# ascentai/diy-gym

Measured on AMD Instinct MI355X. Metric: env steps/sec (whole node), higher is better.
Workload: dtype f32; 1 GPU; ur_high_5 x 16384 envs per GPU; envs_total=16384, substeps=2, auto_reset=True, launch=hipGraph replay of 8-step segments, parallelism=independent env shards x1, no collective, envs_per_wavefront=64, lds_bytes_per_workgroup=160512, parity=vs the C oracle only; parity with pybullet itself is UNPINNED (DESIGN.md 4)

## Files before the change

### diy_gym_amd/backend.py

```python
import collections
import ctypes
import os

import numpy as np
import torch

_HERE = os.path.dirname(os.path.abspath(__file__))
LIB_PATH = os.path.join(_HERE, 'csrc', 'libdiygym_hip.so')

_lib = None

_c_i32p = ctypes.POINTER(ctypes.c_int32)
_c_f64p = ctypes.POINTER(ctypes.c_double)
_vp = ctypes.c_void_p


class JointSelector(ctypes.Structure):
    _fields_ = [('frame', ctypes.c_int32), ('flags', ctypes.c_int32), ('link_mask', ctypes.c_uint64), ('frame_mask', ctypes.c_uint64),
                ('rigid', ctypes.c_float * 10)]


class AccelSelector(ctypes.Structure):
    _fields_ = [('frame', ctypes.c_int32), ('com', ctypes.c_int32), ('pos', ctypes.c_float * 3), ('quat', ctypes.c_float * 4)]

# ... 32 lines not shown
    'dg_world_link_states': (ctypes.c_int32, [_vp, _vp, _c_i32p, _c_i32p, ctypes.c_int32, ctypes.c_int32, _vp, _vp]),
    'dg_world_reset_base_state': (ctypes.c_int32, [_vp, _vp, ctypes.c_int32, _vp, _vp, _vp, _vp, _vp, _vp]),
    'dg_world_joint_wrench': (ctypes.c_int32, [_vp, _vp, ctypes.c_int32, ctypes.POINTER(JointSelector), ctypes.c_int32, _vp, _vp]),
    'dg_world_joint_efforts': (ctypes.c_int32, [_vp, _vp, ctypes.c_int32, _vp, _vp]),
    'dg_world_link_accelerations': (ctypes.c_int32, [_vp, _vp, ctypes.c_int32, ctypes.POINTER(AccelSelector), ctypes.c_int32, _vp, _vp]),
    'dg_world_task_space': (ctypes.c_int32, [_vp, _vp, ctypes.c_int32, ctypes.c_int32, ctypes.POINTER(ctypes.c_float), ctypes.c_int32, _vp, _vp, _vp, _vp,
                                             ctypes.c_float, _vp, _vp, _vp, _vp, _vp, _vp, _vp, _vp]),
    'dg_world_forward_dynamics': (ctypes.c_int32, [_vp, _vp, ctypes.c_int32, _vp, _vp, _vp, ctypes.c_int32, _vp, _vp, _vp]),
    'dg_world_rollout': (ctypes.c_int32, [_vp, _vp, ctypes.c_int32, ctypes.c_int32, ctypes.POINTER(ctypes.c_float), ctypes.c_int32, ctypes.c_int32, ctypes.c_float,
                                          ctypes.c_int32, _vp, _vp, _vp, _vp, _vp, _vp, _vp, _vp]),
    'dg_world_dynamics_derivatives': (ctypes.c_int32, [_vp, _vp, ctypes.c_int32, ctypes.c_int32, _vp, _vp, _vp, ctypes.c_int32, _vp, _vp, _vp, _vp, _vp, _vp, _vp, _vp]),
    'dg_world_rollout_feedback': (ctypes.c_int32, [_vp, _vp, ctypes.c_int32, ctypes.c_int32, ctypes.POINTER(ctypes.c_float), ctypes.c_int32, ctypes.c_int32, ctypes.c_float,
                                                   ctypes.c_int32, _vp, _vp, _vp, _vp, _vp, _vp, _vp, _vp, _vp, _vp, _vp, _vp, _vp, _vp, _vp]),
    'dg_world_inertial_parameters': (ctypes.c_int32, [_vp, _vp, ctypes.c_int32, ctypes.c_int32, _vp, _vp]),
    'dg_world_id_regressor': (ctypes.c_int32, [_vp, _vp, ctypes.c_int32, ctypes.c_int32, _vp, _vp, _vp, _vp, _vp, _vp, _vp, _vp, _vp, _vp]),
    'dg_world_lq_backward': (ctypes.c_int32, [_vp, ctypes.c_int32, ctypes.c_int32, ctypes.c_int32, ctypes.c_int32, ctypes.c_int32, ctypes.c_double,
                                              _vp, _vp, _vp, _vp, _vp, _vp, _vp, _vp, _vp, _vp, _vp, _vp, _vp, _vp, _vp]),
    'dg_world_closest_scratch_floats': (ctypes.c_int64, [_vp]),
    'dg_world_closest': (ctypes.c_int32, [_vp, _vp, ctypes.c_int32, ctypes.c_int32, ctypes.c_int32, ctypes.c_int32, ctypes.c_float, ctypes.c_int32, _vp,
                                          _vp, _vp, _vp, _vp, _vp, _vp]),
    'dg_world_set_render_diag': (ctypes.c_int32, [_vp, ctypes.c_int32]),
    'dg_world_set_diag_buffer': (ctypes.c_int32, [_vp, _vp]),
    'dg_world_set_skip_counter': (ctypes.c_int32, [_vp, _vp]),
    'dg_world_set_profile_buffer': (ctypes.c_int32, [_vp, _vp]),
    'dg_debug_plan': (ctypes.c_int32, [_c_i32p, ctypes.c_int64, _c_f64p, ctypes.c_int64, ctypes.c_int32, ctypes.c_int32, _c_i32p, _c_i32p,
                                       ctypes.c_int64]),
}


def load_library(path=None):
    global _lib
    if _lib is not None and path is None:
        return _lib
    path = path or LIB_PATH
    if not os.path.isfile(path):
        raise RuntimeError('HIP library not built: %s is missing. Run `python -c "import __graft_entry__ as g; g.build()"` '
                           '(or `make -j8 -C diy_gym_amd/csrc`).  There is no CPU fallback.' % path)
    lib = ctypes.CDLL(path)
    for name, (res, args) in SYMBOLS.items():
        fn = getattr(lib, name)
        fn.restype = res
        fn.argtypes = args
    _lib = lib
    return lib


# ... 159 lines not shown
class HipBackend:
    def __init__(self, layout, num_envs, device=None, seed=0, env_index_base=0):
        if not torch.cuda.is_available():
            raise RuntimeError('diy_gym_amd needs a ROCm GPU (torch.cuda.is_available() is False); there is no CPU fallback')
        self.lib = load_library()
        self.layout = layout
        self.num_envs = int(num_envs)
        self.device = torch.device(device if device is not None else 'cuda:0')
        if self.device.type != 'cuda':
            raise RuntimeError('diy_gym_amd runs on ROCm devices only, got %s' % self.device)
        dev_index = self.device.index if self.device.index is not None else torch.cuda.current_device()
        self.device = torch.device('cuda', dev_index)
        self.stride = ((self.num_envs + 63) // 64) * 64
        I, F = layout.I, layout.F
        handle = _vp()
        rc = self.lib.dg_world_create(I.ctypes.data_as(_c_i32p), I.size, F.ctypes.data_as(_c_f64p), F.size, self.num_envs,
                                      self.stride, dev_index, ctypes.c_uint64(seed), ctypes.c_int64(env_index_base),
                                      ctypes.byref(handle))
        self._check(rc)
        self.handle = handle
        dims = (ctypes.c_int32 * 8)()
        self._check(self.lib.dg_world_dims(self.handle, dims))
        self.state_dim, self.act_dim, self.obs_dim, self.rew_dim, self.term_dim, self.n_links, self.lds_bytes, self.lanes = list(dims)
        B, dev = self.num_envs, self.device
        with torch.cuda.device(dev):
            self.state = torch.zeros((self.state_dim, self.stride), dtype=torch.float32, device=dev)
            self.act = torch.zeros((B, max(self.act_dim, 1)), dtype=torch.float32, device=dev)
            self.obs = torch.zeros((B, max(self.obs_dim, 1)), dtype=torch.float32, device=dev)
            self.rew = torch.zeros((B, max(self.rew_dim, 1)), dtype=torch.float32, device=dev)
            self.term = torch.zeros((B, max(self.term_dim, 1)), dtype=torch.uint8, device=dev)
            self.rew_sum = torch.zeros((B, ), dtype=torch.float32, device=dev)
            self.term_flag = torch.zeros((B, ), dtype=torch.uint8, device=dev)
        self._ray_scratch, self._ray_out = None, {}
        self._dyn_out = {}
        self._contact_out = {}
        self._contact_force_out, self._net_contact_out = {}, {}
        self._closest_scratch, self._closest_out = None, {}
        self._closest_k = {}
        self._ik_list_cache = {}
        self._link_states_out = {}
        self._joint_wrench_out = {}
        self._link_accel_out = {}
        self._link_accel_sel = {}
        self._check(self.lib.dg_world_init_state(self.handle, _ptr(self.state), self._stream()))

    def _stream(self):
# ... 918 lines not shown
```

### diy_gym_amd/csrc/dg_api.hip

```cpp
#include <hip/hip_runtime.h>

#include <cmath>
#include <cstdarg>
#include <cstdio>
#include <cstdlib>
#include <cstring>
#include <memory>
#include <string>
#include <vector>

#include "../../include/diygym_hip.h"
#include "dg_launch.h"
#include "dg_plan.h"
#define DG_DEFINE_RENDER_KERNEL
#include "dg_render.h"
#include "dg_raycast.h"
#include "dg_dynq.h"
#include "dg_ikq.h"
#include "dg_jointq.h"
#include "dg_accelq.h"
#include "dg_taskq.h"
#include "dg_fdq.h"
#include "dg_ddq.h"
#include "dg_regq.h"
// ... 192 lines not shown
  if (w->par) snprintf(buf, sizeof buf, "step_kernel_par (4 wavefronts per 64 envs)");
  else snprintf(buf, sizeof buf, "step_kernel<%d>", w->lanes);
  return buf;
}

int32_t dg_world_dims(const dg_world* w, int32_t dims[8]) {
  if (!w || !dims) return fail(DG_ERR_ARG, "null argument");
  dims[0] = w->sc.state_dim; dims[1] = w->sc.act_dim; dims[2] = w->sc.obs_dim; dims[3] = w->sc.rew_dim; dims[4] = w->sc.term_dim;
  dims[5] = w->sc.nl; dims[6] = w->lds_bytes; dims[7] = w->lanes;
  return DG_OK;
}
int32_t dg_world_get_motor_cfg(const dg_world* w, double* cfg) {
  if (!w || !cfg) return fail(DG_ERR_ARG, "null argument");
  for (int k = 0; k < 3 * w->sc.nl; k++) cfg[k] = w->mt.v[k];
  return DG_OK;
}
int32_t dg_world_set_motor_cfg(dg_world* w, const double* cfg) {
  if (!w || !cfg) return fail(DG_ERR_ARG, "null argument");
  for (int k = 0; k < 3 * w->sc.nl; k++) w->mt.v[k] = (float)cfg[k];
  return DG_OK;
}
int32_t dg_world_set_diag_buffer(dg_world* w, int32_t* diag) { if (!w) return fail(DG_ERR_ARG, "null world"); w->diag = diag; return DG_OK; }
int32_t dg_world_set_skip_counter(dg_world* w, int32_t* skipped) { if (!w) return fail(DG_ERR_ARG, "null world"); w->sc.skip_count = skipped; return DG_OK; }

int32_t dg_world_init_state(dg_world* w, float* state, void* stream) {
  if (!w || !state) return fail(DG_ERR_ARG, "null argument");
  DG_ON_DEVICE(w->device);
  hipLaunchKernelGGL(init_state_kernel, dim3((w->stride + 255) / 256), dim3(256), 0, (hipStream_t)stream, w->d_init, state, w->sc.state_dim, w->stride);
  HIP_TRY(hipGetLastError());
  return DG_OK;
}

int32_t dg_world_reset(dg_world* w, float* state, const uint8_t* mask, float* obs, void* stream) {
  if (!w || !state) return fail(DG_ERR_ARG, "null argument");
  if (!(w->par && w->sc.hot_start == 1 && !w->no_par_reset)) return launch(w, stream, &LaunchTable::reset, state, mask, obs);
  DG_ON_DEVICE(w->device);
  launch_table(w->lanes, w->mf).step_par(grid_of(w), w->lds_bytes, (hipStream_t)stream, false, w->sc, w->mt, state, nullptr, 0ull, obs, nullptr, nullptr, nullptr, nullptr, nullptr, nullptr, mask, 1);
  HIP_TRY(hipGetLastError());
  return DG_OK;
}

int32_t dg_world_step(dg_world* w, float* state, const float* actions, uint64_t update_mask, float* obs, float* rew, uint8_t* term,
                      float* rew_sum, uint8_t* term_flag, void* stream) {
  if (!w || !state) return fail(DG_ERR_ARG, "null argument");
  if (w->sc.act_dim > 0 && update_mask != 0 && !actions) return fail(DG_ERR_ARG, "update_mask selects controller addons but actions is NULL");
  DG_ON_DEVICE(w->device);
// ... 649 lines not shown
```

### diy_gym_amd/csrc/dg_kernels.h

```cpp
#pragma once
#include "dg_device.h"
#include "../../include/diygym_scene.h"
#include "../../include/diygym_hip.h"

namespace dg {

#define DG_MAX_LINKS 64
#define DG_MAX_BODIES 192

#define DG_CONSTANT __attribute__((address_space(4)))
typedef const int32_t DG_CONSTANT* cip;
typedef const float DG_CONSTANT* cfp;

struct DevScene {
  cip BI, LI, FI, SI, PI, GI, OI, IL;
  cfp BF, LF, FF, SF, PF, OF, FL, HF;
  cip PLB;
  int split_pgs;
  int early_dyn;
  int coll_split, cont2_off;
  int coll_wave;
  cfp GD;
  cip AM;
  cip SD;
  cip PD;
  cip PLL;
  int32_t nba;
  int32_t no_sliced_reset;
  int32_t no_minv_slices;
  int32_t nsha;
  int32_t debug_keep_ext;
  int32_t no_chain_rows;
  int32_t warm_off;
  float* hull_ws;
  int32_t ncons; cip KI; cfp KF;
  int32_t nb, nl, nfr, nsh, npairs, ngroups, nops, act_dim, obs_dim, rew_dim, term_dim, substeps, iters, hot_start, ik_iters;
  int32_t state_dim, addon_off, max_contacts, term_mode, n_term_groups;
  int32_t tr_off, tr_slots, cont_off, nv_max, total_slots, ab_stride;
  int32_t nt, dv_base, dense;
  int32_t crow_tail;
  int32_t helper_body;
  int32_t reg_body[2];
  int32_t num_envs, stride;
  uint64_t seed; int64_t env_base;
  float h, gx, gy, gz;
  float hm;
  int32_t np_skip;
  cfp RH;
  int32_t* skip_count;
};
struct MotorTable { float v[DG_MAX_LINKS * 3]; };

enum { PLB_R0 = 0, PLB_MINV, PLB_DV, PLB_NV, PLB_CHAIN , PLB_STRIDE };
enum { PLL_POSE = 0, PLL_MROW, PLL_IAACC , PLL_STRIDE };
enum { AW_E = 0, AW_R = 9, AW_V = 12, AW_PA = 18, AW_U = 24, AW_D = 30, AW_UU = 31, AW_STRIDE = 32 };
enum { AB_V = 0, AB_A = 6, AB_FIXED_STRIDE = 12, AB_IA = 12, AB_PA = 33, AB_L = 39, AB_FLOAT_STRIDE = 60 };
enum { CL_PAIR = 0, CL_P = 1, CL_N = 4, CL_DIST = 7, CL_KEY = 8, CL_DVA = 9, CL_NVA = 10, CL_DVB = 11, CL_NVB = 12, CL_MU = 13, CL_STRIDE = 14 };
enum { MR_B = 0, MR_ACC, MR_LO_B, MR_LO_ACC, MR_HI_B, MR_HI_ACC, MR_STRIDE };

constexpr int envs_per_wave(int lanes) { return lanes > 0 ? lanes : (lanes < 0 ? -lanes : 64); }

template <int LANES>
DGD float* workspace_of(const DevScene& sc, float* smem, float* gws, int lane) {
  if constexpr (LANES > 0) return smem + lane;
  else return gws + (size_t)blockIdx.x * (size_t)sc.total_slots * envs_per_wave(LANES) + lane;
}

template <int LANES>
struct Lane {
  const DevScene& sc;
// ... 313 lines not shown
        float rhs[6] = {-p0.a.x, -p0.a.y, -p0.a.z, -p0.l.x, -p0.l.y, -p0.l.z}, x[6];
        if (jdof < 0) {
#pragma unroll
          for (int k = 0; k < 6; k++) rhs[k] = (k == col) ? 1.0f : 0.0f;
        }
        chol6_solve(Lb, rhs, x);
        a0c.a = v3(x[0], x[1], x[2]); a0c.l = v3(x[3], x[4], x[5]);
#pragma unroll
        for (int k = 0; k < 6; k++) L(mo + col * nv + k) = x[k];
      }
      for (int i = 0; i <= jdof; i++) {
        int gl = first + i, par = li(gl)[DG_LI_PARENT]; int o = aw(i);
        S6 ap = par < 0 ? a0c : L6(aw(par - first) + AW_V);
        S6 a1 = xmotion(LM(o + AW_E), L3(o + AW_R), ap);
        float qdd = (L(o + AW_UU) - dot(L6(o + AW_U), a1)) / L(o + AW_D);
        L6set(o + AW_V, a1 + subspace(gl) * qdd);
        L(mo + col * nv + nb6 + i) = qdd;
      }
    }
    for (int r = 0; r < nv; r++) for (int c = r + 1; c < nv; c++) L(mo + r * nv + c) = L(mo + c * nv + r);
    prof.stamp(4 );
  }

  template <int N, class PROF_T>
  DGD void dynamics_chain(int b, PROF_T& prof) const {
    cip B = bi(b); const int first = B[DG_BI_FIRST_LINK], n = B[DG_BI_N_LINKS], mo = plb(b)[PLB_MINV]; const float h = sc.h;
    const M3 R0 = LR(plb(b)[PLB_R0]); const V3 gb = tmul(R0, v3(sc.gx, sc.gy, sc.gz));
    const float ka = ang_damping(b);
    const S6 zero6 = {v3(0.f, 0.f, 0.f), v3(0.f, 0.f, 0.f)};
    M3 E[N]; V3 r[N]; S6 v[N], pA[N], U[N], Sx[N]; float dinv[N], u[N], qd[N];
    S6 vp = zero6;
#pragma unroll
    for (int i = 0; i < N; i++) {
      E[i] = R0; r[i] = v3(0.f, 0.f, 0.f); v[i] = zero6; pA[i] = zero6; U[i] = zero6; Sx[i] = zero6; dinv[i] = 0.f; u[i] = 0.f; qd[i] = 0.f;
      if (i < n) {
        const int gl = first + i, lo = li(gl)[DG_LI_STATE_OFF]; cfp f = lf(gl);
        const float q = S(lo + DG_LS_Q); qd[i] = S(lo + DG_LS_QD);
        M3 Rpc; joint_xform(gl, q, Rpc, r[i]); E[i] = transpose(Rpc); Sx[i] = subspace(gl);
        v[i] = xmotion(E[i], r[i], vp) + Sx[i] * qd[i]; vp = v[i];
        float lm; V3 c; Sym3 Ic; link_inertia(gl, lm, c, Ic); (void)f;
        const AI I = rigid_inertia(lm, c, Ic);
        pA[i] = crf(v[i], mul(I, v[i])) - damping_force(lm, c, Ic, v[i], ka);
      }
    }
    AI carry; bool have = false;
#pragma unroll
    for (int i = N - 1; i >= 0; i--) {
      if (i < n) {
        const int gl = first + i, lo = li(gl)[DG_LI_STATE_OFF]; cfp f = lf(gl);
        const float tau = S(lo + DG_LS_TORQUE) - f[DG_LF_DAMPING] * qd[i];
        AI IA; { float lm; V3 lc; Sym3 lI; link_inertia(gl, lm, lc, lI); IA = rigid_inertia(lm, lc, lI); }
        if (have) {
          IA.I.xx += carry.I.xx; IA.I.xy += carry.I.xy; IA.I.xz += carry.I.xz; IA.I.yy += carry.I.yy; IA.I.yz += carry.I.yz; IA.I.zz += carry.I.zz;
          IA.M.xx += carry.M.xx; IA.M.xy += carry.M.xy; IA.M.xz += carry.M.xz; IA.M.yy += carry.M.yy; IA.M.yz += carry.M.yz; IA.M.zz += carry.M.zz;
#pragma unroll
          for (int k = 0; k < 9; k++) IA.H.m[k] += carry.H.m[k];
        }
        U[i] = mul(IA, Sx[i]); const float d = dot(Sx[i], U[i]); dinv[i] = 1.0f / d; u[i] = tau - dot(Sx[i], pA[i]);
        if (i > 0) {
          const float di = dinv[i]; const S6 Ui = U[i];
          AI Ia = IA;
          Ia.I.xx -= Ui.a.x * Ui.a.x * di; Ia.I.xy -= Ui.a.x * Ui.a.y * di; Ia.I.xz -= Ui.a.x * Ui.a.z * di;
          Ia.I.yy -= Ui.a.y * Ui.a.y * di; Ia.I.yz -= Ui.a.y * Ui.a.z * di; Ia.I.zz -= Ui.a.z * Ui.a.z * di;
          Ia.M.xx -= Ui.l.x * Ui.l.x * di; Ia.M.xy -= Ui.l.x * Ui.l.y * di; Ia.M.xz -= Ui.l.x * Ui.l.z * di;
          Ia.M.yy -= Ui.l.y * Ui.l.y * di; Ia.M.yz -= Ui.l.y * Ui.l.z * di; Ia.M.zz -= Ui.l.z * Ui.l.z * di;
          const float ua[3] = {Ui.a.x, Ui.a.y, Ui.a.z}, ul[3] = {Ui.l.x, Ui.l.y, Ui.l.z};
#pragma unroll
          for (int a = 0; a < 3; a++)
#pragma unroll
            for (int c2 = 0; c2 < 3; c2++) Ia.H.m[3 * a + c2] -= ua[a] * ul[c2] * di;
          const S6 c = crm(v[i], Sx[i] * qd[i]);
          const S6 pa = pA[i] + mul(Ia, c) + Ui * (u[i] * di);
          carry = to_parent(Ia, E[i], r[i]); have = true;
          pA[i - 1] = pA[i - 1] + xforce_to_parent(E[i], r[i], pa);
        }
      }
    }
    S6 ap; ap.a = v3(0.f, 0.f, 0.f); ap.l = -gb;
#pragma unroll
    for (int i = 0; i < N; i++) {
      if (i < n) {
        const S6 a1 = xmotion(E[i], r[i], ap) + crm(v[i], Sx[i] * qd[i]);
        const float qdd = (u[i] - dot(U[i], a1)) * dinv[i];
        ap = a1 + Sx[i] * qdd;
        Sset(li(first + i)[DG_LI_STATE_OFF] + DG_LS_QD, qd[i] + h * qdd);
      }
    }
    prof.stamp(3 );
#pragma unroll
    for (int col = 0; col < N; col++) {
      if (col < n) {
        S6 p[N]; float uu[N];
#pragma unroll
        for (int i = 0; i < N; i++) { p[i] = zero6; uu[i] = 0.f; }
#pragma unroll
        for (int i = col; i >= 0; i--) {
          uu[i] = (i == col ? 1.0f : 0.0f) - dot(Sx[i], p[i]);
          if (i > 0) p[i - 1] = p[i - 1] + xforce_to_parent(E[i], r[i], p[i] + U[i] * (uu[i] * dinv[i]));
        }
        S6 a = zero6;
#pragma unroll
        for (int i = 0; i < N; i++) {
          if (i < n) {
            const S6 a1 = xmotion(E[i], r[i], a);
            const float qdd = (uu[i] - dot(U[i], a1)) * dinv[i];
            a = a1 + Sx[i] * qdd;
            L(mo + col * n + i) = qdd;
          }
        }
      }
    }
// ... 139 lines not shown
```

### diy_gym_amd/csrc/dg_plan.h

```cpp
#pragma once
#include <string>
#include <vector>

#include "dg_kernels.h"

namespace dg {

#define DG_PLAN_SWITCHES(X) \
  X(DG_MAX_LANES, max_lanes, "32|16|8|4|1: envs per wavefront to start from; any value also switches the automatic narrowing off") \
  X(DG_NO_NARROW_MODES, no_narrow_modes, "never below 16 envs per wavefront") \
  X(DG_NO_WAVE_ENV, no_wave_env, "never one env per wavefront") \
  X(DG_NO_SLICED_GLOBAL, no_sliced_global, "global workspace with 64 envs per wavefront instead of 16") \
  X(DG_NO_HELPER_WAVE, no_helper_wave, "single-wavefront step kernel") \
  X(DG_NO_COLLIDE_WAVE, no_collide_wave, "the main wavefront runs the narrow phase itself") \
  X(DG_NO_COLLIDE_SPLIT, no_collide_split, "one narrow-phase wavefront instead of two") \
  X(DG_NO_EARLY_DYNAMICS, no_early_dynamics, "the first substep's dynamics wait for the update ops") \
  X(DG_NO_SPLIT_SWEEPS, no_split_sweeps, "the main wavefront sweeps both arms") \
  X(DG_NO_SPLIT_CONTACTS, no_split_contacts, "contact rows stay on the main wavefront when the sweeps are split") \
  X(DG_NO_REG_ROWS, no_reg_rows, "sliced sweeps keep their rows in LDS") \
  X(DG_NO_FULL_IK, no_full_ik, "the general register-resident IK instead of the packed six-axis solve") \
  X(DG_NO_MINV_SLICES, no_minv_slices, "M^-1 columns by one lane per env") \
  X(DG_NO_CHAIN_ROWS, no_chain_rows, "contact rows between two register-chain bodies pair by pair") \
  X(DG_NO_SLICED_RESET, no_sliced_reset, "masked resets through the one-lane-per-env reset kernel") \
  X(DG_NO_PAR_RESET, no_par_reset, "masked resets of four-wavefront scenes through the one-wavefront reset kernel") \
  X(DG_DEBUG_KEEP_EXT, debug_keep_ext, "external wrenches and joint torques are not cleared at the end of a step") \
  X(DG_RENDER_NO_CULL, render_no_cull, "render: every shape tested for every pixel group (render diag bit 0)") \
  X(DG_RENDER_DIAG, render_diag, "render: initial value of the dg_world_set_render_diag flags") \
  X(DG_RENDER_WPE, render_wpe, "render: 1|3 wavefronts per SIMD builds of the render kernel instead of 2")

struct Switch {
  bool set = false;
  int value = 0;
  explicit operator bool() const { return set; }
};
struct PlanSwitches {
#define X(name, field, doc) Switch field;
  DG_PLAN_SWITCHES(X)
#undef X
  Switch no_np_skip;
};
PlanSwitches plan_switches_from_env();

struct WorldPlan {
  int lanes = 64, lds_bytes = 0;
  bool par = false;
  bool mf = false;
  bool no_par_reset = false;
  int render_diag = 0, render_wpe = 2;
  size_t gws_floats = 0;
  size_t hull_ws_floats = 0;
  std::vector<int32_t> table;
  size_t pd_off = 0, gd_off = 0, sd_off = 0, am_off = 0, rh_off = 0;
  std::vector<int32_t> blob_i;
  std::vector<float> blob_f;
  MotorTable mt;
  std::vector<float> init;
  DevScene sc;
  std::string error;
};

int plan_world(const int32_t* I, int64_t n_i, const double* F, int64_t n_f, int num_envs, int env_stride, int cu_count, uint64_t seed,
               int64_t env_index_base, const PlanSwitches& sw, WorldPlan& out);
// ... 3 lines not shown
```

### diy_gym_amd/csrc/dg_plan.hip

```cpp
#include "dg_plan.h"

#include <algorithm>
#include <cmath>
#include <cstdarg>
#include <cstdio>
#include <cstdlib>
#include <cstring>

#include "dg_solver.h"

namespace dg {

PlanSwitches plan_switches_from_env() {
  PlanSwitches s;
#define X(name, field, doc) if (const char* v = getenv(#name)) { s.field.set = true; s.field.value = atoi(v); }
  DG_PLAN_SWITCHES(X)
#undef X
  if (const char* v = getenv("DG_NO_NP_SKIP")) { s.no_np_skip.set = true; s.no_np_skip.value = atoi(v); }
  return s;
}

namespace {

const int LDS_MAX = 160 * 1024;

const char* check_blob(const int32_t* I, int64_t n_i, int64_t n_f) {
  struct T { int off, count_idx, stride; bool is_f; const char* name; };
  const T tables[] = {
    {DG_H_OFF_BODY_I, DG_H_N_BODIES, DG_BI_STRIDE, false, "body ints"}, {DG_H_OFF_LINK_I, DG_H_N_LINKS, DG_LI_STRIDE, false, "link ints"},
    {DG_H_OFF_FRAME_I, DG_H_N_FRAMES, DG_FI_STRIDE, false, "frame ints"}, {DG_H_OFF_SHAPE_I, DG_H_N_SHAPES, DG_SI_STRIDE, false, "shape ints"},
    {DG_H_OFF_PAIR_I, DG_H_N_PAIRS, DG_PI_STRIDE, false, "pairs"}, {DG_H_OFF_GROUP_I, DG_H_N_GROUPS, DG_GI_STRIDE, false, "pair groups"},
    {DG_H_OFF_CAMERA_I, DG_H_N_CAMERAS, DG_CI_STRIDE, false, "camera ints"}, {DG_H_OFF_OP_I, DG_H_N_OPS, DG_OI_STRIDE, false, "op ints"},
    {DG_H_OFF_ILIST, DG_H_N_ILIST, 1, false, "int list"},
    {DG_H_OFF_BODY_F, DG_H_N_BODIES, DG_BF_STRIDE, true, "body floats"}, {DG_H_OFF_LINK_F, DG_H_N_LINKS, DG_LF_STRIDE, true, "link floats"},
    {DG_H_OFF_FRAME_F, DG_H_N_FRAMES, DG_FF_STRIDE, true, "frame floats"}, {DG_H_OFF_SHAPE_F, DG_H_N_SHAPES, DG_SF_STRIDE, true, "shape floats"},
    {DG_H_OFF_POINT_F, DG_H_N_POINTS, 3, true, "hull points"}, {DG_H_OFF_PLANE_F, DG_H_N_PLANES, 4, true, "hull planes"},
    {DG_H_OFF_CAMERA_F, DG_H_N_CAMERAS, DG_CF_STRIDE, true, "camera floats"}, {DG_H_OFF_OP_F, DG_H_N_OPS, DG_OF_STRIDE, true, "op floats"},
    {DG_H_OFF_FLIST, DG_H_N_FLIST, 1, true, "float list"},
    {DG_H_OFF_CONS_I, DG_H_N_CONSTRAINTS, DG_KI_STRIDE, false, "constraint ints"}, {DG_H_OFF_CONS_F, DG_H_N_CONSTRAINTS, DG_KF_STRIDE, true, "constraint floats"}};
  for (const T& t : tables) {
    const int64_t off = I[t.off], cnt = I[t.count_idx], lim = t.is_f ? n_f : n_i;
// ... 251 lines not shown
    }
  }
  sc.early_dyn = 0;
  if (sc.coll_wave && !sw.no_early_dynamics) {
    bool ok = true, long_update = false;
    for (int op = 0; op < nops; op++) {
      const int32_t* oi = OI + op * DG_OI_STRIDE; const int code = oi[DG_OI_CODE];
      if (code == DG_OP_IK_CONTROL) long_update = true;
      if (code == DG_OP_EXTERNAL_FORCE || code == DG_OP_PROPELLOR || code == DG_OP_ADMITTANCE || (code == DG_OP_JOINT_CONTROL && oi[DG_OI_FLAGS] == DG_JC_TORQUE)) ok = false;
    }
    sc.early_dyn = (ok && long_update) ? 1 : 0;
  }
  sc.np_skip = 0;
  if (sc.coll_wave && sc.coll_split && sc.split_pgs > 0 && ncons == 0 && sc.substeps >= 2 && !sw.no_np_skip && sc.total_slots * 64 * 4 <= LDS_MAX) {
    bool ok = sc.reg_body[0] >= 0 && sc.reg_body[1] == sc.helper_body;
    for (int k = 0; k < 2 && ok; k++) {
      const int32_t* B = BI + sc.reg_body[k] * DG_BI_STRIDE; const int first = B[DG_BI_FIRST_LINK];
      ok = is_fixed(B) && B[DG_BI_N_LINKS] == 6 && PLB[sc.reg_body[k] * PLB_STRIDE + PLB_CHAIN];
      for (int i = 0; i < 6 && ok; i++) ok = LI[(first + i) * DG_LI_STRIDE + DG_LI_TYPE] == 0;
    }
    for (int b = 0; b < nb && ok; b++) if (!is_static(BI + b * DG_BI_STRIDE) && b != sc.reg_body[0] && b != sc.reg_body[1]) ok = false;
    sc.np_skip = ok ? 1 : 0;
  }
  memset(&out.mt, 0, sizeof out.mt);
  for (int l = 0; l < nl; l++) { out.mt.v[3 * l] = 0.f; out.mt.v[3 * l + 1] = 1.f; out.mt.v[3 * l + 2] = -(float)F[DG_HF_DEFAULT_MOTOR_IMPULSE]; }
  for (int op = 0; op < nops; op++) {
    const int32_t* oi = OI + op * DG_OI_STRIDE;
    if (oi[DG_OI_CODE] == DG_OP_ADMITTANCE) for (int k = 0; k < oi[DG_OI_N]; k++) out.mt.v[3 * (I[I[DG_H_OFF_ILIST] + oi[DG_OI_ILIST] + k]) + 2] = 0.f;
  }
  std::vector<float>& init = out.init; init.assign((size_t)sc.state_dim, 0.f);
  const double* BF = F + I[DG_H_OFF_BODY_F];
  for (int b = 0; b < nb; b++) {
    const int so = BI[b * DG_BI_STRIDE + DG_BI_STATE_OFF]; if (so < 0) continue;
    for (int k = 0; k < 3; k++) init[so + DG_BS_POS + k] = (float)BF[b * DG_BF_STRIDE + DG_BF_INIT_POS + k];
    for (int k = 0; k < 4; k++) init[so + DG_BS_QUAT + k] = (float)BF[b * DG_BF_STRIDE + DG_BF_INIT_QUAT + k];
  }
  for (int op = 0; op < nops; op++) {
    const int32_t* oi = OI + op * DG_OI_STRIDE;
    if (oi[DG_OI_CODE] == DG_OP_RANDOMIZE_COLOR) {
      float* tx = init.data() + sc.addon_off + oi[DG_OI_STATE_OFF];
      for (int k = 0; k < 3; k++) tx[DG_TX_A + k] = tx[DG_TX_B + k] = (float)BF[oi[DG_OI_BODY] * DG_BF_STRIDE + DG_BF_COLOR + k];
      tx[DG_TX_FREQ] = 1.f; tx[DG_TX_KIND] = (float)DG_TEX_FLAT;
      continue;
    }
    if (oi[DG_OI_CODE] != DG_OP_RANDOMIZE_DYNAMICS) continue;
    const int so = sc.addon_off + oi[DG_OI_STATE_OFF];
// ... 8 lines not shown
```

### diy_gym_amd/csrc/dg_solver.h

```cpp
#pragma once
#include "dg_kernels.h"
#include "dg_hull.h"

namespace dg {

enum { PS_UPDATE = 0, PS_KIN, PS_COLLIDE, PS_ABA, PS_MINV, PS_ROWS, PS_PGS, PS_INTEGRATE, PS_OUTPUT, PS_PGS_MOTOR, PS_PGS_LIMIT, PS_PGS_CONTACT, PS_COUNT,
       PS_ROW = PS_COUNT + 12  };
template <bool PROF> struct Prof;
template <> struct Prof<false> { DGD void start() {} DGD void stamp(int) {} };
template <> struct Prof<true> {
  unsigned long long last, acc[PS_COUNT];
  DGD void start() { _Pragma("unroll") for (int k = 0; k < PS_COUNT; k++) acc[k] = 0ull; last = __builtin_amdgcn_s_memtime(); }
  DGD void stamp(int id) {
    unsigned long long t = __builtin_amdgcn_s_memtime();
    _Pragma("unroll") for (int k = 0; k < PS_COUNT; k++) if (k == id) acc[k] += t - last;
    last = t;
  }
};

struct WShape { int type, body, glink; M3 R; V3 p; float prm0, prm1, prm2, mu; int poff, npts; };

template <int LANES>
DGD void shape_world(const Lane<LANES>& ln, int sh, WShape& o) {
  cip si = ln.sc.SI + sh * DG_SI_STRIDE; cfp sf = ln.sc.SF + sh * DG_SF_STRIDE;
// ... 1822 lines not shown
template <int LANES>
DGD bool substep_contact_free(const Lane<LANES>& ln) {
  const DevScene& sc = ln.sc;
  if (sc.split_pgs <= 0 || sc.ncons > 0) return false;
  if (ln.bi(sc.reg_body[0])[DG_BI_N_LINKS] != 6 || ln.bi(sc.helper_body)[DG_BI_N_LINKS] != 6) return false;
  float cnt = ln.L(sc.cont_off);
  if (sc.coll_split) cnt = fmaxf(cnt, ln.L(sc.cont2_off));
  return !__any(cnt > 0.f);
}
template <int LANES>
DGD bool substep_np_skip(const Lane<LANES>& ln, bool prev_fused) {
  const DevScene& sc = ln.sc;
  if (!sc.np_skip || !prev_fused) return false;
  const int xo = split_slots(sc);
  const float clr = fminf(ln.L(xo + NPS_CLEAR), ln.L(xo + NPS_CLEAR + 1)), d = ln.L(xo + NPS_MOVE0) + ln.L(xo + NPS_MOVE1);
  return __all(clr > __builtin_fmaf(d, 1.0f + 0x1p-10f, 1e-4f));
}
template <int LANES>
DGD void np_skip_follow(const Lane<LANES>& ln, int which, int list) {
  const int xo = split_slots(ln.sc);
  ln.L(list) = 0.f;
  ln.L(xo + NPS_CLEAR + which) = ln.L(xo + NPS_CLEAR + which) - (ln.L(xo + NPS_MOVE0) + ln.L(xo + NPS_MOVE1));
}
template <int LANES, bool PROF>
DGD void fused_free_halves(const Lane<LANES>& ln, int wave, Prof<PROF>& prof) {
  constexpr int RN = 6;
  const DevScene& sc = ln.sc; const float h = sc.h, lerp = sc.HF[DG_HF_LIMIT_ERP], vmax = sc.HF[DG_HF_MAX_COORD_VEL];
  const float thr_abs = sqrtf(sc.HF[DG_HF_RESIDUAL_THRESHOLD]);
  int lane = threadIdx.x & 63; asm volatile("" : "+v"(lane));
  const int half = lane >> 5, el = (lane & 31) + 32 * wave;
  float* const col = ln.lds - (threadIdx.x & 63) + el;
  const int envl = (int)blockIdx.x * 64 + el; const bool exists = envl < sc.num_envs;
  const bool store = (__ballot(ln.valid) >> el) & 1ull;
  float* const st = ln.st - ln.env + (exists ? envl : sc.num_envs - 1);
  const size_t stride = sc.stride;
  const int b0 = sc.reg_body[0], b1 = sc.helper_body;
  const int f0 = ln.bi(b0)[DG_BI_FIRST_LINK], f1 = ln.bi(b1)[DG_BI_FIRST_LINK];
  const int mvo = half ? ln.plb(b1)[PLB_MINV] : ln.plb(b0)[PLB_MINV];
  const float* const cm = col + (size_t)mvo * 64;
  int lo[RN]; float q[RN], qd[RN], tp[RN], tv[RN];
#pragma unroll
  for (int i = 0; i < RN; i++) {
    const int lo0 = ln.li(f0 + i)[DG_LI_STATE_OFF], lo1 = ln.li(f1 + i)[DG_LI_STATE_OFF]; lo[i] = half ? lo1 : lo0;
    q[i] = st[(lo[i] + DG_LS_Q) * stride]; qd[i] = st[(lo[i] + DG_LS_QD) * stride];
    tp[i] = st[(lo[i] + DG_LS_TARGET_POS) * stride]; tv[i] = st[(lo[i] + DG_LS_TARGET_VEL) * stride];
  }
// ... 89 lines not shown
  uint64_t limit_rows = 0ull;
  const float thr = sc.HF[DG_HF_RESIDUAL_THRESHOLD]; const int rs = crow_stride(sc.crow_tail);
  const bool early = PAR && sc.early_dyn && index == 0;
  constexpr int EPW = envs_per_wave(LANES), SLN = SLICED ? 64 / EPW : 1, SLOG = SLN == 64 ? 6 : SLN == 16 ? 4 : SLN == 8 ? 3 : SLN == 4 ? 2 : SLN == 2 ? 1 : 0;
  const int qlane = threadIdx.x & 63, qsl = qlane & (SLN - 1), qe = qlane >> SLOG;
  const int qenv = blockIdx.x * EPW + qe; const bool qvalid = qenv < sc.num_envs; const int qec = qvalid ? qenv : sc.num_envs - 1;
  const Lane<LANES> lq(sc, ln.mt, SLICED ? ln.lds - qlane + qe : ln.lds, SLICED ? ln.st - ln.env + qec : ln.st, SLICED ? qec : ln.env, SLICED ? qvalid : ln.valid);
  if (primary) {
  if (index == sc.substeps - 1 && !early) for (int b = 0; b < sc.nba; b++) if (b != hb) save_prev_velocities(ln, b);
  if (!early && !(PAR && np_skip)) for (int b = 0; b < sc.nba; b++) if (b != hb) ln.kinematics(b);
  }
  if (PAR) __syncthreads();
  prof.stamp(PS_KIN);
  if constexpr (SLICED) collide<LANES, 64, SLN>(lq, 0, 0x7fffffff, -1, qsl);
  const bool own_collide = !(PAR && sc.coll_wave);
  if (primary) {
  if constexpr (SLICED) ncont = (int)ln.L(sc.cont_off);
  else if (own_collide) ncont = collide<LANES, FULLWAVE ? 64 : (PAR ? 64 : 0)>(ln);
  prof.stamp(PS_COLLIDE);
  }
  if (!early) for (int b = 0; b < sc.nba; b++) {
    if (b == hb || (ln.fixed(b) && ln.bi(b)[DG_BI_N_LINKS] == 0)) continue;
    const int mslices = (SLICED && !ln.plb(b)[PLB_CHAIN] && !sc.no_minv_slices) ? ln.minv_slices(b, SLN) : 0;
    if (primary) { if (ln.plb(b)[PLB_CHAIN]) ln.template dynamics_chain<6>(b, prof); else ln.dynamics(b, prof, mslices > 0); }
    if constexpr (SLICED) { if (mslices > 0) { lq.minv_sliced(b, qsl, mslices, SLN); prof.stamp(4 ); } }
    if (primary) {
      const int dvo = ln.plb(b)[PLB_DV], nv = ln.plb(b)[PLB_NV];
      for (int k = 0; k < nv; k++) ln.L(dvo + k) = 0.f;
    }
  }
  if (primary) {
  if (PAR) __syncthreads();
  if constexpr (PAR) { fused = substep_contact_free(ln); if (fused) fused_free_halves(ln, 0, prof); }
  if (!fused) {
  if (!own_collide) {
    ncont = (int)ln.L(sc.cont_off);
    if (sc.coll_split) {
      const int nb2 = (int)ln.L(sc.cont2_off);
      if (__any(nb2 > 0)) {
        for (int j = 0; j < sc.max_contacts; j++) {
          if (!__any(j < nb2)) break;
          if (j < nb2 && ncont + j < sc.max_contacts) {
            float* dst = ln.lds + (sc.cont_off + 1 + (ncont + j) * CL_STRIDE) * envs_per_wave(LANES);
#pragma unroll
            for (int k = 0; k < CL_KEY + 1; k++) dst[k * envs_per_wave(LANES)] = ln.L(sc.cont2_off + 1 + j * CL_STRIDE + k);
          }
        }
// ... 238 lines not shown
    int32_t* d = diag_out + (size_t)DG_DIAG_STRIDE * ln.env;
    d[DG_DIAG_CONTACTS] = ncont; d[DG_DIAG_PGS_ITERS] = iters_done;
    if (index == 0) { d[DG_DIAG_PGS_ITERS_FIRST] = iters_done; d[DG_DIAG_CONTACTS_FIRST] = ncont; }
  };
  if (primary) {
  store_warm_cache(ln, ncont, wave_max_cont);
  if (diag_out && ln.valid && !fused) write_diag();
  for (int b = 0; b < sc.nba; b++) if (!((split_now || fused) && b == hb) && !(fused && b == sc.reg_body[0])) integrate_body(ln, b);
  }
  if (PAR) __syncthreads();
  if constexpr (PAR) {
    if (fused && diag_out && ln.valid) { iters_done = (int)ln.L(split_slots(sc)); write_diag(); }
  }
  return fused;
}

template <int LANES>
DGD bool helper_substep(const Lane<LANES>& ln, bool early, bool last, bool np_skip) {
  const DevScene& sc = ln.sc; const int hb = sc.helper_body; Prof<false> none;
  if (last && !early) save_prev_velocities(ln, hb);
  if (!early && !np_skip) ln.kinematics(hb);
  __syncthreads();
  if (!early) {
    ln.template dynamics_chain<6>(hb, none);
    const int dvo = ln.plb(hb)[PLB_DV], nv = ln.plb(hb)[PLB_NV]; for (int k = 0; k < nv; k++) ln.L(dvo + k) = 0.f;
  }
  __syncthreads();
  if (substep_contact_free(ln)) { fused_free_halves(ln, 1, none); __syncthreads();  return true; }
  uint64_t lm = 0ull, lr = 0ull;
  if (sc.split_pgs) { const int hf = ln.bi(hb)[DG_BI_FIRST_LINK]; setup_link_rows(ln, hf, hf + ln.bi(hb)[DG_BI_N_LINKS], lm, lr); }
  const int hf0 = ln.bi(hb)[DG_BI_FIRST_LINK];
  if (split_decide_follow(ln, hf0 + 6 <= 32 ? (unsigned)((lr >> (2 * hf0)) & 0xFFFull) : 0u, true)) {
    pgs_reg_halves(ln, 1);
    __syncthreads();
    integrate_body(ln, hb);
  }
  __syncthreads();
  return false;
}

template <int LANES, bool PROF, bool PAR = false, bool SLICED = false, bool FULLWAVE = false>
DGD void sim_step(const Lane<LANES>& ln, int32_t* diag_out, Prof<PROF>& prof, float* smem = nullptr, float* gws = nullptr) {
  const DevScene& sc = ln.sc;
  if constexpr (PAR) {
    bool fused = false; int skipped = 0;
    for (int k = 0; k < sc.substeps; k++) {
      const bool skip = substep_np_skip(ln, fused); skipped += skip ? 1 : 0;
// ... 764 lines not shown
```

### diy_gym_amd/csrc/dg_step_par_body.inc

```
  constexpr int reset_mode = DG_PAR_RESET;
  extern __shared__ float smem[];
  const int wave = threadIdx.x >> 6, lane = threadIdx.x & 63;
  const int env = blockIdx.x * 64 + lane; const bool exists = env < sc.num_envs; const int e = exists ? env : sc.num_envs - 1;
  const bool doit = exists && (!reset_mode || reset_mask == nullptr || reset_mask[e] != 0);
  if (reset_mode && !__any(doit)) return;
  const bool valid = reset_mode ? doit : exists;
  const float* act_row = actions ? actions + (size_t)e * sc.act_dim : nullptr;
  const unsigned long long t_start = PROF ? __builtin_amdgcn_s_memtime() : 0ull; (void)t_start;
  const int clr_slot = split_slots(sc) + NPS_CLEAR;
  const bool pose_ho = sc.early_dyn && sc.coll_split;
  if (wave == 3) {
    Lane<64> ln(sc, mt, smem + lane, state + e, e, valid);
    if (reset_mode) __syncthreads();
    if (pose_ho) ln.kinematics(sc.helper_body, -1, false);
    DG_WAVE_STAMP(0); __syncthreads();
    if (sc.early_dyn) {
      early_dynamics(ln, 1);
      if (sc.coll_split) { float clr; collide<64, 64, 1, true>(ln, sc.npairs / 2, 0x7fffffff, sc.cont2_off, 0, &clr); ln.L(clr_slot + 1) = clr; }
    }
    DG_WAVE_STAMP(1); __syncthreads();
    bool fused = false;
    for (int k = 0; k < sc.substeps; k++) {
      const bool skip = substep_np_skip(ln, fused);
      __syncthreads();
      if (skip) np_skip_follow(ln, 1, sc.cont2_off);
      else if (sc.coll_split && !(sc.early_dyn && k == 0)) { float clr; collide<64, 64, 1, true>(ln, sc.npairs / 2, 0x7fffffff, sc.cont2_off, 0, &clr); ln.L(clr_slot + 1) = clr; }
      __syncthreads();
      fused = substep_contact_free(ln);
      if (!fused && split_decide_follow(ln, 0u, false)) __syncthreads();
      __syncthreads();
    }
    DG_WAVE_STAMP(2); __syncthreads();
    run_output_ops(ln, nullptr, (valid && rew) ? rew + (size_t)e * sc.rew_dim : nullptr, (valid && term) ? term + (size_t)e * sc.term_dim : nullptr,
                   (valid && rew_sum) ? rew_sum + e : nullptr, (valid && term_flag) ? term_flag + e : nullptr, OUT_REW_TERM);
    DG_WAVE_STAMP(3);
    return;
  }
  if (wave == 2) {
    Lane<64> ln(sc, mt, smem + lane, state + e, e, valid);
    if (reset_mode) __syncthreads();
    if (pose_ho) ln.kinematics(sc.reg_body[0], -1, false);
    DG_WAVE_STAMP(0); __syncthreads();
    if (sc.early_dyn) {
      { float clr; collide<64, 64, 1, true>(ln, 0, sc.coll_split ? sc.npairs / 2 : 0x7fffffff, -1, 0, &clr); ln.L(clr_slot) = clr; }
      early_dynamics(ln, 0);
    }
    DG_WAVE_STAMP(1); __syncthreads();
    bool fused = false;
    for (int k = 0; k < sc.substeps; k++) {
      const bool skip = substep_np_skip(ln, fused);
      __syncthreads();
      if (skip) np_skip_follow(ln, 0, sc.cont_off);
      else if (sc.coll_wave && !(sc.early_dyn && k == 0)) { float clr; collide<64, 64, 1, true>(ln, 0, sc.coll_split ? sc.npairs / 2 : 0x7fffffff, -1, 0, &clr); ln.L(clr_slot) = clr; }
      __syncthreads();
      fused = substep_contact_free(ln);
      if (!fused && split_decide_follow(ln, false, false)) __syncthreads();
      __syncthreads();
    }
    DG_WAVE_STAMP(2); __syncthreads();
    run_output_ops(ln, (valid && obs) ? obs + (size_t)e * sc.obs_dim : nullptr, nullptr, nullptr, nullptr, nullptr, OUT_OBS_REST);
    DG_WAVE_STAMP(3);
    return;
  }
  if (wave == 1) {
    Lane<64> ln(sc, mt, smem + lane, state + e, e, valid);
    if (reset_mode) __syncthreads();
    Handover b0([&]() { DG_WAVE_STAMP(0); __syncthreads(); }, false);
    if (pose_ho) ln.base_rot_to_lds(sc.helper_body); else { ln.kinematics(sc.helper_body); b0(); }
    if (act_row) run_update_ops(ln, act_row, mask, sc.helper_body, -1, diag, b0);
    b0();
    DG_WAVE_STAMP(1); __syncthreads();
    bool fused = false;
    for (int k = 0; k < sc.substeps; k++) { const bool skip = substep_np_skip(ln, fused); fused = helper_substep(ln, sc.early_dyn && k == 0, k == sc.substeps - 1, skip); }
    ln.kinematics(sc.helper_body);
    DG_WAVE_STAMP(2); __syncthreads();
// ... 24 lines not shown
```

### include/diygym_hip.h

```cpp
#ifndef DIYGYM_HIP_H
#define DIYGYM_HIP_H
#include <stdint.h>
#ifdef __cplusplus
extern "C" {
#endif

#define DG_OK 0
#define DG_ERR_BAD_SCENE (-1)
#define DG_ERR_HIP (-2)
#define DG_ERR_UNSUPPORTED (-3)
#define DG_ERR_ARG (-4)

typedef struct dg_world dg_world;

int32_t dg_version(void);
const char* dg_last_error(void);

int32_t dg_world_create(const int32_t* idata, int64_t n_i, const double* fdata, int64_t n_f, int32_t num_envs,
                        int32_t env_stride, int32_t device, uint64_t seed, int64_t env_index_base, dg_world** out);

void dg_world_destroy(dg_world* w);

int32_t dg_world_dims(const dg_world* w, int32_t dims[8]);

// ... 131 lines not shown
                                      float* dtau_dq, float* dtau_dqd, int32_t* singular, void* stream);

int32_t dg_world_inertial_parameters(dg_world* w, const float* state, int32_t body, int32_t nominal, float* theta, void* stream);

int32_t dg_world_id_regressor(dg_world* w, const float* state, int32_t body, int32_t P, const float* q, const float* qd, const float* qdd,
                              const float* qd_ref, const float* theta_hat, const float* s, float* Y, float* tau, float* grad, void* stream);

int32_t dg_world_rollout_feedback(dg_world* w, const float* state, int32_t body, int32_t frame, const float* local_pos, int32_t K, int32_t T,
                                  float dt, int32_t joint_damping, const float* q0, const float* qd0, const float* tau_ff, const float* dtau,
                                  const float* alpha, const float* gain, const float* q_ref, const float* qd_ref, const float* tau_limit,
                                  float* q_out, float* qd_out, float* tau_out, float* pos_out, int32_t* singular, void* stream);

int32_t dg_world_lq_backward(dg_world* w, int32_t body, int32_t T, int32_t P, int32_t PC, int32_t substeps, double dt,
                             const float* A_q, const float* A_v, const float* Minv, const float* lxx, const float* luu, const float* lx,
                             const float* lu, const float* lxx_T, const float* lx_T, const float* mu,
                             float* K_out, float* k_out, float* dV, int32_t* status, void* stream);

enum { DG_DIAG_CONTACTS = 0, DG_DIAG_PGS_ITERS = 1, DG_DIAG_PGS_ITERS_FIRST = 2, DG_DIAG_CONTACTS_FIRST = 3, DG_DIAG_IK_ITERS = 4,
       DG_DIAG_N_IK = 4, DG_DIAG_STRIDE = 8 };
int32_t dg_world_set_diag_buffer(dg_world* w, int32_t* diag);

int32_t dg_world_set_skip_counter(dg_world* w, int32_t* skipped);

int32_t dg_world_set_profile_buffer(dg_world* w, uint64_t* cycles);

enum { DG_PLAN_LANES = 0, DG_PLAN_LDS_BYTES, DG_PLAN_PAR, DG_PLAN_MF, DG_PLAN_TOTAL_SLOTS, DG_PLAN_TR_OFF, DG_PLAN_TR_SLOTS, DG_PLAN_CONT_OFF,
       DG_PLAN_CONT2_OFF, DG_PLAN_NV_MAX, DG_PLAN_NT, DG_PLAN_DENSE, DG_PLAN_CROW_TAIL, DG_PLAN_AB_STRIDE, DG_PLAN_HELPER_BODY, DG_PLAN_REG_BODY0,
       DG_PLAN_REG_BODY1, DG_PLAN_COLL_WAVE, DG_PLAN_COLL_SPLIT, DG_PLAN_SPLIT_PGS, DG_PLAN_EARLY_DYN, DG_PLAN_GWS_FLOATS, DG_PLAN_HULL_WS_FLOATS,
       DG_PLAN_NBA, DG_PLAN_NSHA, DG_PLAN_PD_OFF, DG_PLAN_GD_OFF, DG_PLAN_SD_OFF, DG_PLAN_AM_OFF, DG_PLAN_TABLE_WORDS, DG_PLAN_NP_SKIP,
       DG_PLAN_RH_OFF, DG_PLAN_COUNT };
enum { DG_PLAN_PLB_STRIDE = 5, DG_PLAN_PLL_STRIDE = 3 };
int32_t dg_debug_plan(const int32_t* idata, int64_t n_i, const double* fdata, int64_t n_f, int32_t num_envs, int32_t cu_count,
                      int32_t* plan, int32_t* table, int64_t table_cap);

#ifdef __cplusplus
}
#endif
#endif
```

Before: 191.4 million env-steps/s.

## Split mass-matrix inverse computation onto idle waves during no-contact skip path

When the no-contact skip path is active, the primary dynamics chain now skips the Minv column computation. A MINV_ONLY variant of dynamics_chain runs it instead on the waves that would otherwise run collision (the np_skip follow path). This moves serial work off the critical path onto otherwise-idle waves. The cost is recomputing the articulated inertias twice and relying on correct synchronisation between the split paths. It can be disabled with DG_NO_MINV_SPLIT.

```diff
diff --git a/diy_gym_amd/backend.py b/diy_gym_amd/backend.py
--- a/diy_gym_amd/backend.py
+++ b/diy_gym_amd/backend.py
@@ -78,6 +78,7 @@
     'dg_world_set_render_diag': (ctypes.c_int32, [_vp, ctypes.c_int32]),
     'dg_world_set_diag_buffer': (ctypes.c_int32, [_vp, _vp]),
     'dg_world_set_skip_counter': (ctypes.c_int32, [_vp, _vp]),
+    'dg_world_minv_split': (ctypes.c_int32, [_vp]),
     'dg_world_set_profile_buffer': (ctypes.c_int32, [_vp, _vp]),
     'dg_debug_plan': (ctypes.c_int32, [_c_i32p, ctypes.c_int64, _c_f64p, ctypes.c_int64, ctypes.c_int32, ctypes.c_int32, _c_i32p, _c_i32p,
                                        ctypes.c_int64]),
@@ -283,6 +284,7 @@
         dims = (ctypes.c_int32 * 8)()
         self._check(self.lib.dg_world_dims(self.handle, dims))
         self.state_dim, self.act_dim, self.obs_dim, self.rew_dim, self.term_dim, self.n_links, self.lds_bytes, self.lanes = list(dims)
+        self.minv_split = int(self.lib.dg_world_minv_split(self.handle))
         B, dev = self.num_envs, self.device
         with torch.cuda.device(dev):
             self.state = torch.zeros((self.state_dim, self.stride), dtype=torch.float32, device=dev)
diff --git a/diy_gym_amd/csrc/dg_api.hip b/diy_gym_amd/csrc/dg_api.hip
--- a/diy_gym_amd/csrc/dg_api.hip
+++ b/diy_gym_amd/csrc/dg_api.hip
@@ -238,6 +238,7 @@
 }
 int32_t dg_world_set_diag_buffer(dg_world* w, int32_t* diag) { if (!w) return fail(DG_ERR_ARG, "null world"); w->diag = diag; return DG_OK; }
 int32_t dg_world_set_skip_counter(dg_world* w, int32_t* skipped) { if (!w) return fail(DG_ERR_ARG, "null world"); w->sc.skip_count = skipped; return DG_OK; }
+int32_t dg_world_minv_split(const dg_world* w) { return w ? w->sc.minv_split : 0; }
 
 int32_t dg_world_init_state(dg_world* w, float* state, void* stream) {
   if (!w || !state) return fail(DG_ERR_ARG, "null argument");
diff --git a/diy_gym_amd/csrc/dg_kernels.h b/diy_gym_amd/csrc/dg_kernels.h
--- a/diy_gym_amd/csrc/dg_kernels.h
+++ b/diy_gym_amd/csrc/dg_kernels.h
@@ -46,6 +46,7 @@
   float h, gx, gy, gz;
   float hm;
   int32_t np_skip;
+  int32_t minv_split;
   cfp RH;
   int32_t* skip_count;
 };
@@ -405,33 +406,38 @@
     prof.stamp(4 );
   }
 
-  template <int N, class PROF_T>
-  DGD void dynamics_chain(int b, PROF_T& prof) const {
+  template <int N, bool MINV_ONLY = false, class PROF_T>
+  DGD void dynamics_chain(int b, PROF_T& prof, bool with_minv = true) const {
     cip B = bi(b); const int first = B[DG_BI_FIRST_LINK], n = B[DG_BI_N_LINKS], mo = plb(b)[PLB_MINV]; const float h = sc.h;
     const M3 R0 = LR(plb(b)[PLB_R0]); const V3 gb = tmul(R0, v3(sc.gx, sc.gy, sc.gz));
     const float ka = ang_damping(b);
     const S6 zero6 = {v3(0.f, 0.f, 0.f), v3(0.f, 0.f, 0.f)};
-    M3 E[N]; V3 r[N]; S6 v[N], pA[N], U[N], Sx[N]; float dinv[N], u[N], qd[N];
+    constexpr int NV = MINV_ONLY ? 1 : N;
+    M3 E[N]; V3 r[N]; S6 U[N], Sx[N]; float dinv[N];
+    S6 v[NV], pA[NV]; float u[NV], qd[NV];
     S6 vp = zero6;
 #pragma unroll
     for (int i = 0; i < N; i++) {
-      E[i] = R0; r[i] = v3(0.f, 0.f, 0.f); v[i] = zero6; pA[i] = zero6; U[i] = zero6; Sx[i] = zero6; dinv[i] = 0.f; u[i] = 0.f; qd[i] = 0.f;
+      E[i] = R0; r[i] = v3(0.f, 0.f, 0.f); U[i] = zero6; Sx[i] = zero6; dinv[i] = 0.f;
+      if constexpr (!MINV_ONLY) { v[i] = zero6; pA[i] = zero6; u[i] = 0.f; qd[i] = 0.f; }
       if (i < n) {
-        const int gl = first + i, lo = li(gl)[DG_LI_STATE_OFF]; cfp f = lf(gl);
-        const float q = S(lo + DG_LS_Q); qd[i] = S(lo + DG_LS_QD);
+        const int gl = first + i, lo = li(gl)[DG_LI_STATE_OFF];
+        const float q = S(lo + DG_LS_Q);
         M3 Rpc; joint_xform(gl, q, Rpc, r[i]); E[i] = transpose(Rpc); Sx[i] = subspace(gl);
-        v[i] = xmotion(E[i], r[i], vp) + Sx[i] * qd[i]; vp = v[i];
-        float lm; V3 c; Sym3 Ic; link_inertia(gl, lm, c, Ic); (void)f;
-        const AI I = rigid_inertia(lm, c, Ic);
-        pA[i] = crf(v[i], mul(I, v[i])) - damping_force(lm, c, Ic, v[i], ka);
+        if constexpr (!MINV_ONLY) {
+          qd[i] = S(lo + DG_LS_QD);
+          v[i] = xmotion(E[i], r[i], vp) + Sx[i] * qd[i]; vp = v[i];
+          float lm; V3 c; Sym3 Ic; link_inertia(gl, lm, c, Ic);
+          const AI I = rigid_inertia(lm, c, Ic);
+          pA[i] = crf(v[i], mul(I, v[i])) - damping_force(lm, c, Ic, v[i], ka);
+        }
       }
     }
     AI carry; bool have = false;
 #pragma unroll
     for (int i = N - 1; i >= 0; i--) {
       if (i < n) {
-        const int gl = first + i, lo = li(gl)[DG_LI_STATE_OFF]; cfp f = lf(gl);
-        const float tau = S(lo + DG_LS_TORQUE) - f[DG_LF_DAMPING] * qd[i];
+        const int gl = first + i;
         AI IA; { float lm; V3 lc; Sym3 lI; link_inertia(gl, lm, lc, lI); IA = rigid_inertia(lm, lc, lI); }
         if (have) {
           IA.I.xx += carry.I.xx; IA.I.xy += carry.I.xy; IA.I.xz += carry.I.xz; IA.I.yy += carry.I.yy; IA.I.yz += carry.I.yz; IA.I.zz += carry.I.zz;
@@ -439,7 +445,11 @@
 #pragma unroll
           for (int k = 0; k < 9; k++) IA.H.m[k] += carry.H.m[k];
         }
-        U[i] = mul(IA, Sx[i]); const float d = dot(Sx[i], U[i]); dinv[i] = 1.0f / d; u[i] = tau - dot(Sx[i], pA[i]);
+        U[i] = mul(IA, Sx[i]); const float d = dot(Sx[i], U[i]); dinv[i] = 1.0f / d;
+        if constexpr (!MINV_ONLY) {
+          const float tau = S(li(gl)[DG_LI_STATE_OFF] + DG_LS_TORQUE) - lf(gl)[DG_LF_DAMPING] * qd[i];
+          u[i] = tau - dot(Sx[i], pA[i]);
+        }
         if (i > 0) {
           const float di = dinv[i]; const S6 Ui = U[i];
           AI Ia = IA;
@@ -452,24 +462,29 @@
           for (int a = 0; a < 3; a++)
 #pragma unroll
             for (int c2 = 0; c2 < 3; c2++) Ia.H.m[3 * a + c2] -= ua[a] * ul[c2] * di;
-          const S6 c = crm(v[i], Sx[i] * qd[i]);
-          const S6 pa = pA[i] + mul(Ia, c) + Ui * (u[i] * di);
           carry = to_parent(Ia, E[i], r[i]); have = true;
-          pA[i - 1] = pA[i - 1] + xforce_to_parent(E[i], r[i], pa);
-        }
-      }
-    }
-    S6 ap; ap.a = v3(0.f, 0.f, 0.f); ap.l = -gb;
-#pragma unroll
-    for (int i = 0; i < N; i++) {
-      if (i < n) {
-        const S6 a1 = xmotion(E[i], r[i], ap) + crm(v[i], Sx[i] * qd[i]);
-        const float qdd = (u[i] - dot(U[i], a1)) * dinv[i];
-        ap = a1 + Sx[i] * qdd;
-        Sset(li(first + i)[DG_LI_STATE_OFF] + DG_LS_QD, qd[i] + h * qdd);
-      }
-    }
-    prof.stamp(3 );
+          if constexpr (!MINV_ONLY) {
+            const S6 c = crm(v[i], Sx[i] * qd[i]);
+            const S6 pa = pA[i] + mul(Ia, c) + Ui * (u[i] * di);
+            pA[i - 1] = pA[i - 1] + xforce_to_parent(E[i], r[i], pa);
+          }
+        }
+      }
+    }
+    if constexpr (!MINV_ONLY) {
+      S6 ap; ap.a = v3(0.f, 0.f, 0.f); ap.l = -gb;
+#pragma unroll
+      for (int i = 0; i < N; i++) {
+        if (i < n) {
+          const S6 a1 = xmotion(E[i], r[i], ap) + crm(v[i], Sx[i] * qd[i]);
+          const float qdd = (u[i] - dot(U[i], a1)) * dinv[i];
+          ap = a1 + Sx[i] * qdd;
+          Sset(li(first + i)[DG_LI_STATE_OFF] + DG_LS_QD, qd[i] + h * qdd);
+        }
+      }
+      prof.stamp(3 );
+    }
+    if (!MINV_ONLY && !with_minv) { prof.stamp(4 ); return; }
 #pragma unroll
     for (int col = 0; col < N; col++) {
       if (col < n) {
diff --git a/diy_gym_amd/csrc/dg_plan.h b/diy_gym_amd/csrc/dg_plan.h
--- a/diy_gym_amd/csrc/dg_plan.h
+++ b/diy_gym_amd/csrc/dg_plan.h
@@ -38,6 +38,7 @@
   DG_PLAN_SWITCHES(X)
 #undef X
   Switch no_np_skip;
+  Switch no_minv_split;
 };
 PlanSwitches plan_switches_from_env();
 
diff --git a/diy_gym_amd/csrc/dg_plan.hip b/diy_gym_amd/csrc/dg_plan.hip
--- a/diy_gym_amd/csrc/dg_plan.hip
+++ b/diy_gym_amd/csrc/dg_plan.hip
@@ -17,6 +17,7 @@
   DG_PLAN_SWITCHES(X)
 #undef X
   if (const char* v = getenv("DG_NO_NP_SKIP")) { s.no_np_skip.set = true; s.no_np_skip.value = atoi(v); }
+  if (const char* v = getenv("DG_NO_MINV_SPLIT")) { s.no_minv_split.set = true; s.no_minv_split.value = atoi(v); }
   return s;
 }
 
@@ -314,6 +315,7 @@
     for (int b = 0; b < nb && ok; b++) if (!is_static(BI + b * DG_BI_STRIDE) && b != sc.reg_body[0] && b != sc.reg_body[1]) ok = false;
     sc.np_skip = ok ? 1 : 0;
   }
+  sc.minv_split = (sc.np_skip && !sw.no_minv_split) ? 1 : 0;
   memset(&out.mt, 0, sizeof out.mt);
   for (int l = 0; l < nl; l++) { out.mt.v[3 * l] = 0.f; out.mt.v[3 * l + 1] = 1.f; out.mt.v[3 * l + 2] = -(float)F[DG_HF_DEFAULT_MOTOR_IMPULSE]; }
   for (int op = 0; op < nops; op++) {
diff --git a/diy_gym_amd/csrc/dg_solver.h b/diy_gym_amd/csrc/dg_solver.h
--- a/diy_gym_amd/csrc/dg_solver.h
+++ b/diy_gym_amd/csrc/dg_solver.h
@@ -1868,6 +1868,13 @@
   ln.L(list) = 0.f;
   ln.L(xo + NPS_CLEAR + which) = ln.L(xo + NPS_CLEAR + which) - (ln.L(xo + NPS_MOVE0) + ln.L(xo + NPS_MOVE1));
 }
+template <int LANES>
+DGD void minv_split_follow(const Lane<LANES>& ln, int which) {
+  if (!ln.sc.minv_split) return;
+  Prof<false> none;
+  int b = which ? ln.sc.helper_body : ln.sc.reg_body[0]; asm volatile("" : "+s"(b));
+  ln.template dynamics_chain<6, true>(b, none);
+}
 template <int LANES, bool PROF>
 DGD void fused_free_halves(const Lane<LANES>& ln, int wave, Prof<PROF>& prof) {
   constexpr int RN = 6;
@@ -2003,7 +2010,7 @@
   if (!early) for (int b = 0; b < sc.nba; b++) {
     if (b == hb || (ln.fixed(b) && ln.bi(b)[DG_BI_N_LINKS] == 0)) continue;
     const int mslices = (SLICED && !ln.plb(b)[PLB_CHAIN] && !sc.no_minv_slices) ? ln.minv_slices(b, SLN) : 0;
-    if (primary) { if (ln.plb(b)[PLB_CHAIN]) ln.template dynamics_chain<6>(b, prof); else ln.dynamics(b, prof, mslices > 0); }
+    if (primary) { if (ln.plb(b)[PLB_CHAIN]) ln.template dynamics_chain<6>(b, prof, !(PAR && np_skip && sc.minv_split)); else ln.dynamics(b, prof, mslices > 0); }
     if constexpr (SLICED) { if (mslices > 0) { lq.minv_sliced(b, qsl, mslices, SLN); prof.stamp(4 ); } }
     if (primary) {
       const int dvo = ln.plb(b)[PLB_DV], nv = ln.plb(b)[PLB_NV];
@@ -2288,7 +2295,7 @@
   if (!early && !np_skip) ln.kinematics(hb);
   __syncthreads();
   if (!early) {
-    ln.template dynamics_chain<6>(hb, none);
+    ln.template dynamics_chain<6>(hb, none, !(np_skip && sc.minv_split));
     const int dvo = ln.plb(hb)[PLB_DV], nv = ln.plb(hb)[PLB_NV]; for (int k = 0; k < nv; k++) ln.L(dvo + k) = 0.f;
   }
   __syncthreads();
diff --git a/diy_gym_amd/csrc/dg_step_par_body.inc b/diy_gym_amd/csrc/dg_step_par_body.inc
--- a/diy_gym_amd/csrc/dg_step_par_body.inc
+++ b/diy_gym_amd/csrc/dg_step_par_body.inc
@@ -23,7 +23,7 @@
     for (int k = 0; k < sc.substeps; k++) {
       const bool skip = substep_np_skip(ln, fused);
       __syncthreads();
-      if (skip) np_skip_follow(ln, 1, sc.cont2_off);
+      if (skip) { np_skip_follow(ln, 1, sc.cont2_off); minv_split_follow(ln, 1); }
       else if (sc.coll_split && !(sc.early_dyn && k == 0)) { float clr; collide<64, 64, 1, true>(ln, sc.npairs / 2, 0x7fffffff, sc.cont2_off, 0, &clr); ln.L(clr_slot + 1) = clr; }
       __syncthreads();
       fused = substep_contact_free(ln);
@@ -50,7 +50,7 @@
     for (int k = 0; k < sc.substeps; k++) {
       const bool skip = substep_np_skip(ln, fused);
       __syncthreads();
-      if (skip) np_skip_follow(ln, 0, sc.cont_off);
+      if (skip) { np_skip_follow(ln, 0, sc.cont_off); minv_split_follow(ln, 0); }
       else if (sc.coll_wave && !(sc.early_dyn && k == 0)) { float clr; collide<64, 64, 1, true>(ln, 0, sc.coll_split ? sc.npairs / 2 : 0x7fffffff, -1, 0, &clr); ln.L(clr_slot) = clr; }
       __syncthreads();
       fused = substep_contact_free(ln);
diff --git a/include/diygym_hip.h b/include/diygym_hip.h
--- a/include/diygym_hip.h
+++ b/include/diygym_hip.h
@@ -177,6 +177,8 @@
 
 int32_t dg_world_set_skip_counter(dg_world* w, int32_t* skipped);
 
+int32_t dg_world_minv_split(const dg_world* w);
+
 int32_t dg_world_set_profile_buffer(dg_world* w, uint64_t* cycles);
 
 enum { DG_PLAN_LANES = 0, DG_PLAN_LDS_BYTES, DG_PLAN_PAR, DG_PLAN_MF, DG_PLAN_TOTAL_SLOTS, DG_PLAN_TR_OFF, DG_PLAN_TR_SLOTS, DG_PLAN_CONT_OFF,
```

Result: faster. 201.3 million env-steps/s (median of 6 runs) (+5.2%).
